# pdh930105/ARCQuant

Hardware: AMD Instinct MI355X
Metric: ARC-NVFP4 GEMM TFLOP/s (M=4096, N=KQ=4096, KE=64) (higher is better)
Workload: dtype f16

## Files before the change

### arcquant_amd/csrc/gemm_tile.hip

```cpp
#include <hip/hip_runtime.h>
#include <stdint.h>
#include <stdlib.h>

#include <type_traits>

#include "arcq_internal.hpp"
#include "gemm_common.hpp"
#include "gemm_tile_common.hpp"

namespace arcq {

#ifdef ARCQ_STREAM_STAMPS
static unsigned long long* g_tile_stamps = nullptr;
#ifndef ARCQ_TILE_REPACKED_UNIT
extern "C" void arcq_debug_set_tile_stamps(void* p) { g_tile_stamps = reinterpret_cast<unsigned long long*>(p); }
#endif
#define ARCQ_TILE_STAMP(k)                                                                                     \
  do {                                                                                                         \
    if (p.stamps && tid == 0) {                                                                                \
      unsigned long long t0_, t1_;                                                                             \
      asm volatile("s_memtime %0\n\ts_memrealtime %1\n\ts_waitcnt lgkmcnt(0)" : "=s"(t0_), "=s"(t1_)::"memory"); \
      p.stamps[(size_t)blockIdx.x * (2 * kTileStamps) + 2 * (k)] = t0_;                                        \
      p.stamps[(size_t)blockIdx.x * (2 * kTileStamps) + 2 * (k) + 1] = t1_;                                    \
    }                                                                                                          \
  } while (0)
#else
#define ARCQ_TILE_STAMP(k) do { } while (0)
#endif

#ifndef ARCQ_TILE_WIDE_STORES
#define ARCQ_TILE_WIDE_STORES 1
#endif

template <int BM, int BN, int WAVES_M, int WAVES_N, bool kMfma32, int kEpi, bool kStagger, bool kPipe, int kBLayout = kBRef>
__global__ __launch_bounds__(WAVES_M* WAVES_N * 64) void gemm_tile_kernel(TileParams p) {
  constexpr int kThreads = WAVES_M * WAVES_N * 64;
  constexpr int WM = BM / WAVES_M, WN = BN / WAVES_N;
  constexpr int kT = kMfma32 ? 32 : 16;
  constexpr int TM = WM / kT, TN = WN / kT;
  using acc_t = typename std::conditional<kMfma32, f32x16, f32x4>::type;
  constexpr int A_UNITS = (BM * 2 + kThreads - 1) / kThreads, B_UNITS = (BN * 2 + kThreads - 1) / kThreads;
  constexpr bool A_PARTIAL = (BM * 2) % kThreads != 0, B_PARTIAL = (BN * 2) % kThreads != 0;
  static_assert(!A_PARTIAL || A_UNITS == 1, "a partial A pass is a single pass");
  static_assert(!B_PARTIAL || B_UNITS == 1, "a partial B pass is a single pass");
  constexpr int A_TILE = BM * kRowBytes, B_TILE = BN * kRowBytes;

  extern __shared__ __attribute__((aligned(16))) unsigned char smem[];
  unsigned char* const lds_a0 = smem;
  unsigned char* const lds_b0 = smem + A_TILE;
  unsigned char* const lds_a1 = smem + A_TILE + B_TILE;
  unsigned char* const lds_b1 = smem + 2 * A_TILE + B_TILE;

  const int ntiles = p.tiles_m * p.tiles_n;
  int bid = blockIdx.x, split = 0;
  if (p.splits > 1) {
    split = bid / ntiles;
    bid -= split * ntiles;
  }
  {
    const int q8 = ntiles >> 3, r8 = ntiles & 7, x = bid & 7, j = bid >> 3;
    bid = (x < r8 ? x * (q8 + 1) : r8 * (q8 + 1) + (x - r8) * q8) + j;
  }
  constexpr int kGroupM = 8;
  const int per_group = kGroupM * p.tiles_n;
  const int grp = bid / per_group;
  const int first_m = grp * kGroupM;
  const int gsz = min(p.tiles_m - first_m, kGroupM);
  const int tm = first_m + (bid % per_group) % gsz;
  const int tn = (bid % per_group) / gsz;
  const int m0 = __builtin_amdgcn_readfirstlane(tm * BM), n0 = __builtin_amdgcn_readfirstlane(tn * BN);

  const int tid = threadIdx.x;
  const int lane = tid & 63, wave = tid >> 6;
  const int wr = wave / WAVES_N, wc = wave % WAVES_N;
  ARCQ_TILE_STAMP(0);
  const int half_k = p.K >> 1, atoms_k = p.K >> 6;
  const int a_begin = split * p.atoms_per_split, a_end = min(atoms_k, a_begin + p.atoms_per_split);

  const uint8_t* a_q[A_UNITS];
  const uint8_t* a_sf[A_UNITS];
  uint32_t a_live[A_UNITS];
  int a_slot[A_UNITS][4];
#pragma unroll
  for (int u = 0; u < A_UNITS; ++u) {
    const int unit = tid + u * kThreads, r = A_PARTIAL ? min(unit >> 1, BM - 1) : unit >> 1, h = unit & 1;
    const int row = m0 + r, rc = row < p.M ? row : p.M - 1;
    a_q[u] = p.A + (size_t)rc * half_k + h * 16;
    a_sf[u] = p.SFA + sf_atom_offset(rc, 0, atoms_k) + h * 2;
    a_live[u] = row < p.M ? 0xffffu : 0u;
#pragma unroll
    for (int j = 0; j < 4; ++j) a_slot[u][j] = kMfma32 ? lds_slot32(r, h * 4 + j) : lds_slot(r, h * 4 + j);
  }
  const uint8_t* b_q[B_UNITS];
  const uint8_t* b_sf[B_UNITS];
  uint32_t b_live[B_UNITS];
  int b_slot[B_UNITS][4];
#pragma unroll
  for (int u = 0; u < B_UNITS; ++u) {
    const int unit = tid + u * kThreads, r = B_PARTIAL ? min(unit >> 1, BN - 1) : unit >> 1, h = unit & 1;
    const int row = n0 + r, rc = row < p.N ? row : p.N - 1;
    if constexpr (kBLayout == kBRepacked) {
      const int tiles = ((p.K + 255) >> 8) * 2;
      b_q[u] = p.B + (size_t)(rc >> 4) * tiles * 1024 + h * 256 + (rc & 15) * 16;
      b_sf[u] = p.SFB + (size_t)(rc >> 4) * tiles * 128 + h * 64 + (rc & 15) * 4;
    } else {
      b_q[u] = p.B + (size_t)rc * half_k + h * 16;
      b_sf[u] = p.SFB + sf_atom_offset(rc, 0, atoms_k) + h * 2;
    }
    b_live[u] = row < p.N ? 0xffffu : 0u;
#pragma unroll
    for (int j = 0; j < 4; ++j) b_slot[u][j] = kMfma32 ? lds_slot32(r, h * 4 + j) : lds_slot(r, h * 4 + j);
  }
  const int fa_base = kMfma32 ? lds_slot32(wr * WM + (lane & 31), lane >> 5) : lds_slot(wr * WM + (lane & 15), lane >> 4);
  const int fb_base = kMfma32 ? lds_slot32(wc * WN + (lane & 31), lane >> 5) : lds_slot(wc * WN + (lane & 15), lane >> 4);
  acc_t acc[TM][TN];
#pragma unroll
  for (int i = 0; i < TM; ++i)
#pragma unroll
    for (int j = 0; j < TN; ++j)
#pragma unroll
      for (int r = 0; r < (kMfma32 ? 16 : 4); ++r) acc[i][j][r] = 0.f;

  Staged sa[A_UNITS], sb[B_UNITS];
  auto load_step = [&](int atom) {
#pragma unroll
    for (int u = 0; u < A_UNITS; ++u) sa[u] = stage_load(a_q[u], a_sf[u], atom);
#pragma unroll
    for (int u = 0; u < B_UNITS; ++u) sb[u] = kBLayout == kBRepacked ? stage_load_rw(b_q[u], b_sf[u], atom) : stage_load(b_q[u], b_sf[u], atom);
  };
  auto store_step = [&](unsigned char* la, unsigned char* lb) {
#pragma unroll
    for (int u = 0; u < A_UNITS; ++u)
      if (!A_PARTIAL || tid < BM * 2) stage_store(la, a_slot[u], sa[u], a_live[u]);
#pragma unroll
    for (int u = 0; u < B_UNITS; ++u)
      if (!B_PARTIAL || tid < BN * 2) stage_store(lb, b_slot[u], sb[u], b_live[u]);
  };
  auto mma_step = [&](const unsigned char* la, const unsigned char* lb) {
    if constexpr (kMfma32) {
#pragma unroll
      for (int ks = 0; ks < 4; ++ks) {
        Frag8 fa[TM], fb[TN];
#pragma unroll
        for (int i = 0; i < TM; ++i) fa[i].u = *reinterpret_cast<const uint4*>(la + (fa_base ^ (ks * 32)) + i * 32 * kRowBytes);
#pragma unroll
        for (int j = 0; j < TN; ++j) fb[j].u = *reinterpret_cast<const uint4*>(lb + (fb_base ^ (ks * 32)) + j * 32 * kRowBytes);
#pragma unroll
        for (int i = 0; i < TM; ++i)
#pragma unroll
          for (int j = 0; j < TN; ++j) acc[i][j] = __builtin_amdgcn_mfma_f32_32x32x16_f16(fb[j].v, fa[i].v, acc[i][j], 0, 0, 0);
      }
    } else {
#pragma unroll
      for (int ks = 0; ks < 2; ++ks) {
        Frag8 fa[TM], fb[TN];
#pragma unroll
        for (int i = 0; i < TM; ++i) fa[i].u = *reinterpret_cast<const uint4*>(la + (fa_base ^ (ks * 64)) + i * 16 * kRowBytes);
#pragma unroll
        for (int j = 0; j < TN; ++j) fb[j].u = *reinterpret_cast<const uint4*>(lb + (fb_base ^ (ks * 64)) + j * 16 * kRowBytes);
#pragma unroll
        for (int i = 0; i < TM; ++i)
#pragma unroll
          for (int j = 0; j < TN; ++j) acc[i][j] = __builtin_amdgcn_mfma_f32_16x16x32_f16(fb[j].v, fa[i].v, acc[i][j], 0, 0, 0);
      }
    }
  };
  const bool late = kStagger && wave >= 4;
  auto k_step = [&](int kt, unsigned char* ca, unsigned char* cb, unsigned char* na, unsigned char* nb) {
    Staged ta[A_UNITS], tb[B_UNITS];
#pragma unroll
    for (int u = 0; u < A_UNITS; ++u) ta[u] = sa[u];
#pragma unroll
    for (int u = 0; u < B_UNITS; ++u) tb[u] = sb[u];
    load_step(min(kt + 2 + (late ? 1 : 0), a_end - 1));
    __builtin_amdgcn_sched_barrier(0);
    mma_step(ca, cb);
    if (kStagger && late) __syncthreads();
    unsigned char* const wa = late ? ca : na;
    unsigned char* const wb = late ? cb : nb;
#pragma unroll
    for (int u = 0; u < A_UNITS; ++u)
      if (!A_PARTIAL || tid < BM * 2) stage_store(wa, a_slot[u], ta[u], a_live[u]);
#pragma unroll
    for (int u = 0; u < B_UNITS; ++u)
      if (!B_PARTIAL || tid < BN * 2) stage_store(wb, b_slot[u], tb[u], b_live[u]);
    if (!kStagger || !late) __syncthreads();
  };

  auto k_step_pipe = [&](int kt, unsigned char* ca, unsigned char* cb, unsigned char* na, unsigned char* nb) {
    static_assert(kMfma32 || TM % 2 == 0, "pairs of A fragments");
    Staged ta[A_UNITS], tb[B_UNITS];
#pragma unroll
    for (int u = 0; u < A_UNITS; ++u) ta[u] = sa[u];
#pragma unroll
    for (int u = 0; u < B_UNITS; ++u) tb[u] = sb[u];
    load_step(min(kt + 2, a_end - 1));
    __builtin_amdgcn_sched_barrier(0);
    constexpr int kPieces = (A_UNITS + B_UNITS) * 4, kBlocks = kMfma32 ? 4 : TM;
    auto pieces = [&](int blk) {
#pragma unroll
      for (int c = blk; c < kPieces; c += kBlocks) {
        const int u = c >> 2, j = c & 3;
        if (u < A_UNITS) {
#ifdef ARCQ_EXPERIMENT_A_RAW
          if (!A_PARTIAL || tid < BM * 2) stage_piece_raw(na, a_slot[u < A_UNITS ? u : 0][j], ta[u < A_UNITS ? u : 0], a_live[u < A_UNITS ? u : 0], j);
#else
          if (!A_PARTIAL || tid < BM * 2) stage_piece(na, a_slot[u < A_UNITS ? u : 0][j], ta[u < A_UNITS ? u : 0], a_live[u < A_UNITS ? u : 0], j);
#endif
        } else {
          const int v = u - A_UNITS < B_UNITS ? u - A_UNITS : 0;
#ifdef ARCQ_EXPERIMENT_B_RAW
          if (!B_PARTIAL || tid < BN * 2) stage_piece_raw(nb, b_slot[v][j], tb[v], b_live[v], j);
#else
          if (!B_PARTIAL || tid < BN * 2) stage_piece(nb, b_slot[v][j], tb[v], b_live[v], j);
#endif
        }
      }
    };
    if constexpr (kMfma32) {
      Frag8 f32a[2][TM], f32b[2][TN];
      auto rd_set = [&](int buf, int ks) {
#pragma unroll
        for (int i = 0; i < TM; ++i) f32a[buf][i].u = *reinterpret_cast<const uint4*>(ca + (fa_base ^ (ks * 32)) + i * 32 * kRowBytes);
#pragma unroll
        for (int j = 0; j < TN; ++j) f32b[buf][j].u = *reinterpret_cast<const uint4*>(cb + (fb_base ^ (ks * 32)) + j * 32 * kRowBytes);
      };
      rd_set(0, 0);
#pragma unroll
      for (int ks = 0; ks < 4; ++ks) {
        if (ks + 1 < 4) rd_set((ks + 1) & 1, ks + 1);
        __builtin_amdgcn_sched_barrier(0);
#pragma unroll
        for (int i = 0; i < TM; ++i)
#pragma unroll
          for (int j = 0; j < TN; ++j)
            if constexpr (kMfma32)
              acc[i][j] = __builtin_amdgcn_mfma_f32_32x32x16_f16(f32b[ks & 1][j].v, f32a[ks & 1][i].v, acc[i][j], 0, 0, 0);
        pieces(ks);
        __builtin_amdgcn_sched_barrier(0);
      }
      __syncthreads();
      return;
    }
    auto rd_a = [&](int ks, int i) { Frag8 f; f.u = *reinterpret_cast<const uint4*>(ca + (fa_base ^ (ks * 64)) + i * 16 * kRowBytes); return f; };
    auto rd_b = [&](int ks, int j) { Frag8 f; f.u = *reinterpret_cast<const uint4*>(cb + (fb_base ^ (ks * 64)) + j * 16 * kRowBytes); return f; };
    constexpr int kPairs = TM / 2, kSeq = 2 * kPairs, kAhead = 1;
    Frag8 fb[2][TN], fq[kSeq][2];
    auto rd_pair = [&](int q) {
      fq[q][0] = rd_a(q / kPairs, 2 * (q % kPairs));
      fq[q][1] = rd_a(q / kPairs, 2 * (q % kPairs) + 1);
    };
#pragma unroll
    for (int j = 0; j < TN; ++j) fb[0][j] = rd_b(0, j);
#pragma unroll
    for (int q = 0; q < kAhead; ++q) rd_pair(q);
#pragma unroll
    for (int q = 0; q < kSeq; ++q) {
      const int ks = q / kPairs, pr = q % kPairs;
      if (q + kAhead < kSeq) rd_pair(q + kAhead);
      if (ks == 0 && pr == kPairs - 1 - (kAhead - 1 < kPairs - 1 ? kAhead - 1 : kPairs - 1)) {
#pragma unroll
        for (int j = 0; j < TN; ++j) fb[1][j] = rd_b(1, j);
      }
      __builtin_amdgcn_sched_barrier(0);
#pragma unroll
      for (int ii = 0; ii < 2; ++ii)
#pragma unroll
        for (int j = 0; j < TN; ++j)
          if constexpr (!kMfma32)
            acc[2 * pr + ii][j] = __builtin_amdgcn_mfma_f32_16x16x32_f16(fb[ks][j].v, fq[q][ii].v, acc[2 * pr + ii][j], 0, 0, 0);
      pieces(q);
#pragma unroll
      for (int m8 = 0; m8 < (TM == 8 ? 2 * TN : 0); ++m8) {
        __builtin_amdgcn_sched_group_barrier(0x008, 1, 0);
        __builtin_amdgcn_sched_group_barrier(0x002, 2, 0);
      }
      __builtin_amdgcn_sched_barrier(0);
    }
    __syncthreads();
  };

  load_step(a_begin);
  Staged sa0[A_UNITS], sb0[B_UNITS];
#pragma unroll
  for (int u = 0; u < A_UNITS; ++u) sa0[u] = sa[u];
#pragma unroll
  for (int u = 0; u < B_UNITS; ++u) sb0[u] = sb[u];
  load_step(min(a_begin + 1, a_end - 1));
  __builtin_amdgcn_sched_barrier(0);
#pragma unroll
  for (int u = 0; u < A_UNITS; ++u)
    if (!A_PARTIAL || tid < BM * 2) stage_store(lds_a0, a_slot[u], sa0[u], a_live[u]);
#pragma unroll
  for (int u = 0; u < B_UNITS; ++u)
    if (!B_PARTIAL || tid < BN * 2) stage_store(lds_b0, b_slot[u], sb0[u], b_live[u]);
  if (kStagger && late) {
    store_step(lds_a1, lds_b1);
    load_step(min(a_begin + 2, a_end - 1));
  }
  __syncthreads();
  int kt = a_begin;
#ifndef ARCQ_EXPERIMENT_GENERAL_EPILOGUE
  float alpha_dev = 1.0f;
  if (p.alpha_dev) alpha_dev = *reinterpret_cast<const __attribute__((address_space(4))) float*>(reinterpret_cast<uintptr_t>(p.alpha_dev));
  asm volatile("" : "+s"(alpha_dev));
#endif
  if (WAVES_M * WAVES_N == 8 && wave >= 4) __builtin_amdgcn_s_setprio(1);
  ARCQ_TILE_STAMP(1);
  if constexpr (kPipe) {
    for (; kt + 1 < a_end; kt += 2) {
      k_step_pipe(kt, lds_a0, lds_b0, lds_a1, lds_b1);
      k_step_pipe(kt + 1, lds_a1, lds_b1, lds_a0, lds_b0);
    }
    if (kt < a_end) k_step_pipe(kt, lds_a0, lds_b0, lds_a1, lds_b1);
  } else {
    for (; kt + 1 < a_end; kt += 2) {
      k_step(kt, lds_a0, lds_b0, lds_a1, lds_b1);
      k_step(kt + 1, lds_a1, lds_b1, lds_a0, lds_b0);
    }
    if (kt < a_end) k_step(kt, lds_a0, lds_b0, lds_a1, lds_b1);
  }
  ARCQ_TILE_STAMP(2);

#ifdef ARCQ_EXPERIMENT_GENERAL_EPILOGUE
  const float alpha = p.alpha_host * (p.alpha_dev ? *p.alpha_dev : 1.0f);
#else
  const float alpha = p.alpha_host * alpha_dev;
#endif
  const bool vec_ok = (p.N & 3) == 0;
  uint32_t act_max = 0;
  [[maybe_unused]] auto interior_epilogue = [&](auto has_bias, auto has_res) __attribute__((always_inline)) {
    constexpr bool kBias = decltype(has_bias)::value, kRes = decltype(has_res)::value;
    constexpr bool kSilu = kEpi == kEpiSiluMul;
    constexpr uint32_t kElem = kSilu ? 1 : 2;
    unsigned char* const tile_d = reinterpret_cast<unsigned char*>(p.D) + ((size_t)m0 * p.N + n0) * kElem;
    const unsigned char* const tile_r = kRes ? reinterpret_cast<const unsigned char*>(p.residual) + ((size_t)m0 * p.N + n0) * 2 : nullptr;
    uint32_t t = tid;
    asm volatile("" : "+v"(t));
    const uint32_t lane_row = (t >> 6) / WAVES_N * WM + (t & 15), lane_col = (t >> 6) % WAVES_N * WN + 4 * ((t >> 4) & 3);
    uint32_t off = lane_row * (uint32_t)p.N + lane_col;
    const uint32_t row_step = 16u * (uint32_t)p.N;
    constexpr bool kWide = ARCQ_TILE_WIDE_STORES && !kSilu && TN % 2 == 0;
    typedef uint32_t u32x4_a8 __attribute__((ext_vector_type(4), aligned(8)));
    [[maybe_unused]] const uint32_t g4 = (t >> 4) & 3;
    [[maybe_unused]] uint32_t off_w = off - 4 * g4 + ((g4 & 1) ? 16 + 4 * (g4 - 1) : 4 * g4);
    [[maybe_unused]] uint2 held = make_uint2(0, 0);
    float bias_f[TN][4];
    if constexpr (kBias) {
#pragma unroll
      for (int j = 0; j < TN; ++j) {
        const uint2 b = *reinterpret_cast<const uint2*>(p.bias + n0 + lane_col + j * 16);
        bias_f[j][0] = bf16_bits_to_f32(b.x & 0xffffu); bias_f[j][1] = bf16_bits_to_f32(b.x >> 16);
        bias_f[j][2] = bf16_bits_to_f32(b.y & 0xffffu); bias_f[j][3] = bf16_bits_to_f32(b.y >> 16);
      }
    }
    uint2 res_cur[TN], res_nxt[TN];
    auto res_load = [&](uint32_t o, uint2 (&r)[TN]) {
#pragma unroll
      for (int j = 0; j < TN; ++j) r[j] = *reinterpret_cast<const uint2*>(tile_r + (size_t)o * 2 + j * 32);
    };
    if constexpr (kRes) res_load(off, res_cur);
#pragma unroll
    for (int i = 0; i < TM; ++i) {
      if constexpr (kRes) { if (i + 1 < TM) res_load(off + row_step, res_nxt); }
#pragma unroll
      for (int j = 0; j < TN; ++j) {
        float d[4] = {alpha * acc[i][j][0], alpha * acc[i][j][1], alpha * acc[i][j][2], alpha * acc[i][j][3]};
        if constexpr (kSilu) {
          if constexpr (kBias) {
#pragma unroll
            for (int r = 0; r < 4; r += 2) {
              round2_to_bf16(d[r], d[r + 1]);
              d[r] += bias_f[j][r];
              d[r + 1] += bias_f[j][r + 1];
            }
          }
          const uint32_t y01 = pack_bf16x2_hw(d[0], d[1]), y23 = pack_bf16x2_hw(d[2], d[3]);
          const uint32_t a0 = silu_mul_bf16(y01 & 0xffffu, y01 >> 16), a1 = silu_mul_bf16(y23 & 0xffffu, y23 >> 16);
          *reinterpret_cast<uint32_t*>(tile_d + (size_t)off + j * 16) = a0 | (a1 << 16);
          act_max = max(act_max, max(a0 & 0x7fffu, a1 & 0x7fffu));
        } else {
          if constexpr (kBias) {
#pragma unroll
            for (int r = 0; r < 4; r += 2) {
              round2_to_bf16(d[r], d[r + 1]);
              d[r] += bias_f[j][r];
              d[r + 1] += bias_f[j][r + 1];
            }
          }
          if constexpr (kRes) {
            const uint32_t rw[2] = {res_cur[j].x, res_cur[j].y};
#pragma unroll
            for (int r = 0; r < 4; r += 2) {
              round2_to_bf16(d[r], d[r + 1]);
              d[r] += bf16_bits_to_f32(rw[r >> 1] & 0xffffu);
              d[r + 1] += bf16_bits_to_f32(rw[r >> 1] >> 16);
            }
          }
          const uint2 pk = make_uint2(pack_bf16x2_hw(d[0], d[1]), pack_bf16x2_hw(d[2], d[3]));
          if constexpr (kWide) {
            if (j & 1) {
              const auto lo = __builtin_amdgcn_permlane16_swap(held.x, pk.x, false, false);
              const auto hi = __builtin_amdgcn_permlane16_swap(held.y, pk.y, false, false);
              const u32x4_a8 v = {lo[0], hi[0], lo[1], hi[1]};
              *reinterpret_cast<u32x4_a8*>(tile_d + (size_t)off_w * 2 + (j >> 1) * 64) = v;
            } else {
              held = pk;
            }
          } else {
            *reinterpret_cast<uint2*>(tile_d + (size_t)off * 2 + j * 32) = pk;
          }
        }
        if (i == 0 && j == 0) ARCQ_TILE_STAMP(3);
      }
      if constexpr (kRes) {
#pragma unroll
        for (int j = 0; j < TN; ++j) res_cur[j] = res_nxt[j];
      }
      off += row_step;
      off_w += row_step;
    }
  };
  auto store4 = [&](int m, int n, float d0, float d1, float d2, float d3, bool pre, uint2 bias2, uint2 res2) __attribute__((always_inline)) {
    if (m >= p.M || n >= p.N) return;
    const uint32_t bw[2] = {bias2.x, bias2.y}, rw[2] = {res2.x, res2.y};
    auto bias_at = [&](int r) { return bf16_bits_to_f32(pre ? (bw[r >> 1] >> (16 * (r & 1))) & 0xffffu : (uint32_t)p.bias[n + r]); };
    if (kEpi == kEpiSiluMul) {
      uint32_t y[4] = {f32_to_bf16_bits(alpha * d0), f32_to_bf16_bits(alpha * d1), f32_to_bf16_bits(alpha * d2), f32_to_bf16_bits(alpha * d3)};
      if (p.bias) {
#pragma unroll
        for (int e = 0; e < 4; ++e) y[e] = f32_to_bf16_bits(bf16_bits_to_f32(y[e]) + bias_at(e));
      }
      const uint32_t a0 = silu_mul_bf16(y[0], y[1]);
      const uint32_t a1 = silu_mul_bf16(y[2], y[3]);
      *reinterpret_cast<uint32_t*>(reinterpret_cast<uint16_t*>(p.D) + (size_t)m * (p.N >> 1) + (n >> 1)) = a0 | (a1 << 16);
      act_max = max(act_max, max(a0 & 0x7fffu, a1 & 0x7fffu));
      return;
    }
    if (p.splits > 1) {
      *reinterpret_cast<float4*>(p.partial + ((size_t)split * p.M + m) * p.N + n) = make_float4(d0, d1, d2, d3);
      return;
    }
    float d[4] = {alpha * d0, alpha * d1, alpha * d2, alpha * d3};
    if (p.bias) {
#pragma unroll
      for (int r = 0; r < 4; ++r)
        if (pre || n + r < p.N) d[r] = (p.out_dtype == ARCQ_OUT_F32 ? d[r] : bf16_bits_to_f32(f32_to_bf16_bits(d[r]))) + bias_at(r);
    }
    if (p.residual) {
#pragma unroll
      for (int r = 0; r < 4; ++r)
        if (pre || n + r < p.N) {
          const float res = bf16_bits_to_f32(pre ? (rw[r >> 1] >> (16 * (r & 1))) & 0xffffu : (uint32_t)p.residual[(size_t)m * p.N + n + r]);
          d[r] = (p.out_dtype == ARCQ_OUT_F32 ? d[r] : bf16_bits_to_f32(f32_to_bf16_bits(d[r]))) + res;
        }
    }
    if (p.out_dtype == ARCQ_OUT_F32) {
      float* o = reinterpret_cast<float*>(p.D) + (size_t)m * p.N + n;
      if (vec_ok) *reinterpret_cast<float4*>(o) = make_float4(d[0], d[1], d[2], d[3]);
      else for (int r = 0; r < 4; ++r) if (n + r < p.N) o[r] = d[r];
    } else {
      uint16_t* o = reinterpret_cast<uint16_t*>(p.D) + (size_t)m * p.N + n;
      if (vec_ok) *reinterpret_cast<uint2*>(o) = make_uint2(pack_bf16x2(d[0], d[1]), pack_bf16x2(d[2], d[3]));
      else for (int r = 0; r < 4; ++r) if (n + r < p.N) o[r] = (uint16_t)f32_to_bf16_bits(d[r]);
    }
  };
#ifdef ARCQ_EXPERIMENT_GENERAL_EPILOGUE
  constexpr bool kInteriorPath = false;
#else
  constexpr bool kInteriorPath = !kMfma32;
#endif
  bool interior = false;
  if constexpr (kInteriorPath)
    interior = m0 + BM <= p.M && n0 + BN <= p.N && vec_ok && p.splits <= 1 && p.out_dtype == ARCQ_OUT_BF16 && (int64_t)BM * p.N < (1ll << 31) &&
               ((reinterpret_cast<uintptr_t>(p.bias) | reinterpret_cast<uintptr_t>(p.residual)) & 7) == 0;
  if (interior) {
    if constexpr (kInteriorPath) {
      using T = std::true_type;
      using F = std::false_type;
      if constexpr (kEpi == kEpiSiluMul) {
        if (p.bias) interior_epilogue(T{}, F{});
        else interior_epilogue(F{}, F{});
      } else if (p.bias) {
        if (p.residual) interior_epilogue(T{}, T{});
        else interior_epilogue(T{}, F{});
      } else {
        if (p.residual) interior_epilogue(F{}, T{});
        else interior_epilogue(F{}, F{});
      }
    }
  } else if constexpr (kMfma32) {
#pragma unroll
    for (int i = 0; i < TM; ++i)
#pragma unroll
      for (int j = 0; j < TN; ++j) {
        const int m = m0 + wr * WM + i * 32 + (lane & 31);
#pragma unroll
        for (int g = 0; g < 4; ++g) {
          const int n = n0 + wc * WN + j * 32 + 8 * g + 4 * (lane >> 5);
          store4(m, n, acc[i][j][4 * g + 0], acc[i][j][4 * g + 1], acc[i][j][4 * g + 2], acc[i][j][4 * g + 3], false, make_uint2(0, 0), make_uint2(0, 0));
        }
      }
  } else {
    const bool pre = vec_ok && p.splits <= 1 && ((reinterpret_cast<uintptr_t>(p.bias) | reinterpret_cast<uintptr_t>(p.residual)) & 7) == 0;
    const int nb = n0 + wc * WN + 4 * (lane >> 4), mb = m0 + wr * WM + (lane & 15);
    if (pre) {
      uint2 bias_v[TN], res_cur[TN], res_nxt[TN];
#pragma unroll
      for (int j = 0; j < TN; ++j) {
        bias_v[j] = res_cur[j] = res_nxt[j] = make_uint2(0, 0);
        if (p.bias && nb + j * 16 < p.N) bias_v[j] = *reinterpret_cast<const uint2*>(p.bias + nb + j * 16);
      }
      auto res_load = [&](int i, uint2 (&r)[TN]) {
        if (!p.residual) return;
        const int m = mb + i * 16;
#pragma unroll
        for (int j = 0; j < TN; ++j)
          if (m < p.M && nb + j * 16 < p.N) r[j] = *reinterpret_cast<const uint2*>(p.residual + (size_t)m * p.N + nb + j * 16);
      };
      res_load(0, res_cur);
#pragma unroll
      for (int i = 0; i < TM; ++i) {
        if (i + 1 < TM) res_load(i + 1, res_nxt);
#pragma unroll
        for (int j = 0; j < TN; ++j) {
          store4(mb + i * 16, nb + j * 16, acc[i][j][0], acc[i][j][1], acc[i][j][2], acc[i][j][3], true, bias_v[j], res_cur[j]);
          if (i == 0 && j == 0) ARCQ_TILE_STAMP(3);
        }
#pragma unroll
        for (int j = 0; j < TN; ++j) res_cur[j] = res_nxt[j];
      }
    } else {
#pragma unroll
      for (int i = 0; i < TM; ++i)
#pragma unroll
        for (int j = 0; j < TN; ++j) {
          store4(mb + i * 16, nb + j * 16, acc[i][j][0], acc[i][j][1], acc[i][j][2], acc[i][j][3], false, make_uint2(0, 0), make_uint2(0, 0));
          if (i == 0 && j == 0) ARCQ_TILE_STAMP(3);
        }
    }
  }
  ARCQ_TILE_STAMP(4);
  if (kEpi == kEpiSiluMul) {
    __shared__ uint32_t wave_max[WAVES_M * WAVES_N];
#pragma unroll
    for (int sh = 32; sh > 0; sh >>= 1) act_max = max(act_max, (uint32_t)__shfl_down((int)act_max, sh, 64));
    if (lane == 0) wave_max[wave] = act_max;
    __syncthreads();
    if (tid == 0) {
      uint32_t m = 0;
#pragma unroll
      for (int w = 0; w < WAVES_M * WAVES_N; ++w) m = max(m, wave_max[w]);
      p.slots[blockIdx.x] = m;
    }
  }
}

struct TileCfg { int id, bm, bn, waves; };
static constexpr TileCfg kTileCfgs[] = {{1, 128, 128, 4}, {2, 256, 256, 4}, {3, 256, 256, 8}, {4, 128, 256, 4}, {5, 256, 256, 8}, {6, 128, 128, 4},
                                        {7, 64, 256, 4}, {8, 32, 256, 4}, {9, 128, 128, 4}, {10, 128, 256, 8}, {11, 256, 128, 8}, {12, 128, 128, 8},
                                        {13, 64, 256, 8}, {14, 64, 128, 8}, {15, 64, 64, 4}, {16, 64, 128, 4}, {17, 128, 64, 4}};
static const TileCfg& tile_cfg(int id) {
  for (const TileCfg& c : kTileCfgs)
    if (c.id == id) return c;
  return kTileCfgs[2];
}

static int env_int(const char* name, int dflt) {
  const char* e = getenv(name);
  return e ? atoi(e) : dflt;
}
static int tile_cfg_override() {
  static const int v = env_int("ARCQ_TILE_CFG", 0);
  return v;
}
static int tile_split_override() {
  static const int v = env_int("ARCQ_TILE_SPLIT", 0);
  return v;
}
static bool tile_stagger() {
  static const int v = env_int("ARCQ_TILE_STAGGER", 0);
  return v != 0;
}
static bool tile_pipe() {
  static const int v = env_int("ARCQ_TILE_PIPE", 1);
  return v != 0;
}

static void tile_split(int64_t M, int64_t N, int64_t K, int BM, int BN, int* splits, int* atoms_per_split) {
  const int64_t tiles = ((M + BM - 1) / BM) * ((N + BN - 1) / BN);
  const int atoms = (int)(K / 64);
  int s = 1;
  if ((N % 4) == 0) {
    if (tile_split_override() > 0) s = min(tile_split_override(), max(atoms / 2, 1));
    else
      while (tiles * s < 256 && atoms / (s * 2) >= 8 && s < 32) s *= 2;
  }
  const int per = (atoms + s - 1) / s;
  *splits = (atoms + per - 1) / per;
  *atoms_per_split = per;
}

template <int BM, int BN, int WAVES_M, int WAVES_N, bool kMfma32 = false, int kEpi = kEpiPlain, int kBLayout = kBRef>
static int launch_tile(const GemmArgs& a, hipStream_t stream, bool allow_split = false) {
  TileParams p;
  p.A = a.A; p.B = a.B; p.SFA = a.SFA; p.SFB = a.SFB; p.D = a.D;
  p.alpha_dev = a.alpha_dev; p.bias = a.bias; p.residual = a.residual;
  p.M = a.M; p.N = a.N; p.K = a.K; p.alpha_host = a.alpha_host; p.out_dtype = a.out_dtype;
  p.tiles_m = (a.M + BM - 1) / BM;
  p.tiles_n = (a.N + BN - 1) / BN;
  p.splits = 1; p.atoms_per_split = a.K / 64; p.partial = nullptr;
  p.epi = a.epilogue; p.slots = a.absmax_slots;
#ifdef ARCQ_STREAM_STAMPS
  p.stamps = g_tile_stamps;
#endif
  if (allow_split && a.epilogue == kEpiPlain) {
    tile_split(a.M, a.N, a.K, BM, BN, &p.splits, &p.atoms_per_split);
    if (p.splits > 1) {
      const int64_t need = (int64_t)p.splits * a.M * a.N * (int64_t)sizeof(float);
      if (!a.workspace || a.workspace_bytes < need)
        return fail(ARCQ_ERR_WORKSPACE, "arcq_gemm_nvfp4: split-K needs %lld B of workspace, got %lld", (long long)need,
                    (long long)a.workspace_bytes);
      p.partial = reinterpret_cast<float*>(a.workspace);
    }
  }
  const size_t lds = 2 * (size_t)(BM + BN) * kRowBytes;
  constexpr bool kCanStagger = WAVES_M * WAVES_N == 8 && BM == 256 && BN == 256, kCanPipe = true;
  auto kern = gemm_tile_kernel<BM, BN, WAVES_M, WAVES_N, kMfma32, kEpi, false, false, kBLayout>;
  if (kCanPipe && tile_pipe()) kern = gemm_tile_kernel<BM, BN, WAVES_M, WAVES_N, kMfma32, kEpi, false, kCanPipe, kBLayout>;
  else if (kCanStagger && tile_stagger()) kern = gemm_tile_kernel<BM, BN, WAVES_M, WAVES_N, kMfma32, kEpi, kCanStagger, false, kBLayout>;
  static LdsOptIn lds_opt[3];
  const int which = (kCanPipe && tile_pipe()) ? 1 : (kCanStagger && tile_stagger()) ? 2 : 0;
  if (int rc = ensure_dynamic_lds(reinterpret_cast<const void*>(kern), lds_opt[which], (int)lds, "arcq_gemm_nvfp4 (tile)")) return rc;
  hipLaunchKernelGGL(kern, dim3((unsigned)(p.tiles_m * p.tiles_n * p.splits)), dim3(WAVES_M * WAVES_N * 64), lds, stream, p);
  hipError_t e = hipGetLastError();
  if (e != hipSuccess) return fail(ARCQ_ERR_LAUNCH, "arcq_gemm_nvfp4 (tile): launch failed: %s", hipGetErrorString(e));
  if (p.splits > 1) return gemm_splitk_finish(a, p.splits, stream);
  return ARCQ_OK;
}

static int tile_choice(int64_t M, int64_t N, int64_t K) {
  const int64_t t256 = ((M + 255) / 256) * ((N + 255) / 256);
  if (t256 >= 192) return 3;
  if (M <= 32) return 8;
  if (M <= 64) return 7;
  const int64_t t10 = ((M + 127) / 128) * ((N + 255) / 256);
  if (t10 <= 64 || t10 == 128 || (t10 > 224 && t10 <= 256) || (K >= 8192 && t10 >= 96 && t10 <= 256)) return 10;
  return 1;
}

static int effective_cfg(int64_t M, int64_t N, int64_t K, bool* may_split) {
  int id = tile_cfg_override();
  if (id == 0) id = tile_choice(M, N, K);
  id = tile_cfg(id).id;
  *may_split = !(id >= 2 && id <= 6) && id != 9;
  return id;
}

#ifndef ARCQ_TILE_REPACKED_UNIT
int64_t gemm_tile_silu_slots(int64_t M, int64_t N, int64_t K) {
  bool sp;
  const TileCfg& c = tile_cfg(effective_cfg(M, N, K, &sp));
  return ((M + c.bm - 1) / c.bm) * ((N + c.bn - 1) / c.bn);
}

int64_t gemm_tile_workspace_bytes(int64_t M, int64_t N, int64_t K) {
  int s = 1, per = 0;
  bool sp;
  const TileCfg& c = tile_cfg(effective_cfg(M, N, K, &sp));
  if (sp) tile_split(M, N, K, c.bm, c.bn, &s, &per);
  return s > 1 ? (int64_t)s * M * N * (int64_t)sizeof(float) : 0;
}
#endif

template <int kEpi, int kBLayout>
static int gemm_tile_epi(const GemmArgs& a, hipStream_t stream) {
  bool sp;
  switch (effective_cfg(a.M, a.N, a.K, &sp)) {
    case 1: case 9: return launch_tile<128, 128, 2, 2, false, kEpi, kBLayout>(a, stream, sp);
    case 2: return launch_tile<256, 256, 2, 2, false, kEpi, kBLayout>(a, stream);
    case 4: return launch_tile<128, 256, 2, 2, false, kEpi, kBLayout>(a, stream);
    case 5: return launch_tile<256, 256, 2, 4, true, kEpi, kBLayout>(a, stream);
    case 6: return launch_tile<128, 128, 2, 2, true, kEpi, kBLayout>(a, stream);
    case 7: return launch_tile<64, 256, 1, 4, false, kEpi, kBLayout>(a, stream, sp);
    case 8: return launch_tile<32, 256, 1, 4, false, kEpi, kBLayout>(a, stream, sp);
    case 10: return launch_tile<128, 256, 2, 4, false, kEpi, kBLayout>(a, stream, sp);
    case 11: return launch_tile<256, 128, 4, 2, false, kEpi, kBLayout>(a, stream, sp);
    case 12: return launch_tile<128, 128, 2, 4, false, kEpi, kBLayout>(a, stream, sp);
    case 13: return launch_tile<64, 256, 1, 8, false, kEpi, kBLayout>(a, stream, sp);
    case 14: return launch_tile<64, 128, 2, 4, false, kEpi, kBLayout>(a, stream, sp);
    case 15: return launch_tile<64, 64, 2, 2, false, kEpi, kBLayout>(a, stream, sp);
    case 16: return launch_tile<64, 128, 2, 2, false, kEpi, kBLayout>(a, stream, sp);
    case 17: return launch_tile<128, 64, 2, 2, false, kEpi, kBLayout>(a, stream, sp);
    default: return launch_tile<256, 256, 2, 4, false, kEpi, kBLayout>(a, stream);
  }
}

#ifndef ARCQ_TILE_REPACKED_UNIT
int gemm_tile(const GemmArgs& a, hipStream_t stream) {
  if (a.b_layout == kBRepacked) return gemm_tile_repacked(a, stream);
  return a.epilogue == kEpiSiluMul ? gemm_tile_epi<kEpiSiluMul, kBRef>(a, stream) : gemm_tile_epi<kEpiPlain, kBRef>(a, stream);
}
#else
int gemm_tile_repacked(const GemmArgs& a, hipStream_t stream) {
  return a.epilogue == kEpiSiluMul ? gemm_tile_epi<kEpiSiluMul, kBRepacked>(a, stream) : gemm_tile_epi<kEpiPlain, kBRepacked>(a, stream);
}
#endif

}
```

### arcquant_amd/csrc/gemm_tile_common.hpp

```cpp
#pragma once
#include <hip/hip_runtime.h>
#include <stdint.h>

#include "arcq_internal.hpp"
#include "gemm_common.hpp"

namespace arcq {

struct TileParams {
  const uint8_t* A;
  const uint8_t* B;
  const uint8_t* SFA;
  const uint8_t* SFB;
  void* D;
  const float* alpha_dev;
  const uint16_t* bias;
  const uint16_t* residual;
  int M, N, K;
  float alpha_host;
  int out_dtype;
  int tiles_m, tiles_n;
  int splits, atoms_per_split;
  float* partial;
  int epi;
  unsigned int* slots;
#ifdef ARCQ_STREAM_STAMPS
  unsigned long long* stamps;
#endif
};
constexpr int kTileStamps = 5;

constexpr int kBK = 64;
constexpr int kRowBytes = kBK * 2;

__device__ __forceinline__ int lds_slot(int r, int ks) { return r * kRowBytes + ((ks ^ (r & 7)) << 4); }
__device__ __forceinline__ int lds_slot32(int r, int ks) { return r * kRowBytes + ((ks ^ ((r >> 1) & 7)) << 4); }

struct Staged {
  uint4 q;
  uint32_t sf;
};

__device__ __forceinline__ Staged stage_load(const uint8_t* __restrict__ qrow, const uint8_t* __restrict__ sfrow, int atom) {
  Staged s;
  s.q = *reinterpret_cast<const uint4*>(qrow + (size_t)atom * 32);
  s.sf = *reinterpret_cast<const uint16_t*>(sfrow + (size_t)atom * 512);
  return s;
}

__device__ __forceinline__ Staged stage_load_rw(const uint8_t* __restrict__ qrow, const uint8_t* __restrict__ sfrow, int atom) {
  Staged s;
  s.q = *reinterpret_cast<const uint4*>(qrow + (size_t)atom * 512);
  s.sf = *reinterpret_cast<const uint16_t*>(sfrow + (atom >> 2) * 256 + (atom & 1) * 128 + ((atom >> 1) & 1) * 2);
  return s;
}

__device__ __forceinline__ void stage_piece(unsigned char* tile, int slot, const Staged& s, uint32_t live_mask, int j) {
  const uint32_t w = j == 0 ? s.q.x : j == 1 ? s.q.y : j == 2 ? s.q.z : s.q.w;
  const Frag8 f = dequant8(w, sf_pair_at(s.sf & live_mask, j < 2 ? 0 : 8));
  *reinterpret_cast<uint4*>(tile + slot) = f.u;
}

#if defined(ARCQ_EXPERIMENT_A_RAW) || defined(ARCQ_EXPERIMENT_B_RAW)
__device__ __forceinline__ void stage_piece_raw(unsigned char* tile, int slot, const Staged& s, uint32_t live_mask, int j) {
  const uint32_t w = (j == 0 ? s.q.x : j == 1 ? s.q.y : j == 2 ? s.q.z : s.q.w) & (live_mask | (live_mask << 16)) & 0x3bff3bffu;
  *reinterpret_cast<uint4*>(tile + slot) = make_uint4(w, w, w, w);
}
#endif

__device__ __forceinline__ void stage_store(unsigned char* tile, const int (&slot)[4], const Staged& s, uint32_t live_mask) {
  const uint32_t sf = s.sf & live_mask;
  const f16x2 s0 = sf_pair_at(sf, 0), s1 = sf_pair_at(sf, 8);
  Frag8 f0 = dequant8(s.q.x, s0), f1 = dequant8(s.q.y, s0), f2 = dequant8(s.q.z, s1), f3 = dequant8(s.q.w, s1);
  *reinterpret_cast<uint4*>(tile + slot[0]) = f0.u;
  *reinterpret_cast<uint4*>(tile + slot[1]) = f1.u;
  *reinterpret_cast<uint4*>(tile + slot[2]) = f2.u;
  *reinterpret_cast<uint4*>(tile + slot[3]) = f3.u;
}


}
```

Measured before the change: 1404.

## Peel K-loop tail steps to drop redundant loads, stores and barriers

Restructures the main K loop for the non-stagger paths so the last two iterations are peeled into NoLoad and Last variants. The steady-state step no longer clamps the prefetch atom with min(), the NoLoad step skips global prefetch, and the Last step skips LDS staging and the trailing barrier. This removes wasted loads, dequant stores and a sync at the end of each tile. It also adds asm register pins so the scale-factor mask and fragment offsets are not rematerialized. The cost is more code, since several step variants are inlined, which may raise instruction-cache or register pressure.

```diff
diff --git a/arcquant_amd/csrc/gemm_tile.hip b/arcquant_amd/csrc/gemm_tile.hip
--- a/arcquant_amd/csrc/gemm_tile.hip
+++ b/arcquant_amd/csrc/gemm_tile.hip
@@ -136,15 +136,15 @@
     for (int u = 0; u < B_UNITS; ++u)
       if (!B_PARTIAL || tid < BN * 2) stage_store(lb, b_slot[u], sb[u], b_live[u]);
   };
-  auto mma_step = [&](const unsigned char* la, const unsigned char* lb) {
+  auto mma_step = [&](const unsigned char* la, const unsigned char* lb, int fa_off, int fb_off) {
     if constexpr (kMfma32) {
 #pragma unroll
       for (int ks = 0; ks < 4; ++ks) {
         Frag8 fa[TM], fb[TN];
 #pragma unroll
-        for (int i = 0; i < TM; ++i) fa[i].u = *reinterpret_cast<const uint4*>(la + (fa_base ^ (ks * 32)) + i * 32 * kRowBytes);
-#pragma unroll
-        for (int j = 0; j < TN; ++j) fb[j].u = *reinterpret_cast<const uint4*>(lb + (fb_base ^ (ks * 32)) + j * 32 * kRowBytes);
+        for (int i = 0; i < TM; ++i) fa[i].u = *reinterpret_cast<const uint4*>(la + (fa_off ^ (ks * 32)) + i * 32 * kRowBytes);
+#pragma unroll
+        for (int j = 0; j < TN; ++j) fb[j].u = *reinterpret_cast<const uint4*>(lb + (fb_off ^ (ks * 32)) + j * 32 * kRowBytes);
 #pragma unroll
         for (int i = 0; i < TM; ++i)
 #pragma unroll
@@ -155,9 +155,9 @@
       for (int ks = 0; ks < 2; ++ks) {
         Frag8 fa[TM], fb[TN];
 #pragma unroll
-        for (int i = 0; i < TM; ++i) fa[i].u = *reinterpret_cast<const uint4*>(la + (fa_base ^ (ks * 64)) + i * 16 * kRowBytes);
-#pragma unroll
-        for (int j = 0; j < TN; ++j) fb[j].u = *reinterpret_cast<const uint4*>(lb + (fb_base ^ (ks * 64)) + j * 16 * kRowBytes);
+        for (int i = 0; i < TM; ++i) fa[i].u = *reinterpret_cast<const uint4*>(la + (fa_off ^ (ks * 64)) + i * 16 * kRowBytes);
+#pragma unroll
+        for (int j = 0; j < TN; ++j) fb[j].u = *reinterpret_cast<const uint4*>(lb + (fb_off ^ (ks * 64)) + j * 16 * kRowBytes);
 #pragma unroll
         for (int i = 0; i < TM; ++i)
 #pragma unroll
@@ -165,16 +165,30 @@
       }
     }
   };
+  constexpr int kSteady = 0, kNoLoad = 1, kLast = 2;
+  using Steady = std::integral_constant<int, kSteady>;
+  using NoLoad = std::integral_constant<int, kNoLoad>;
+  using Last = std::integral_constant<int, kLast>;
+  auto next_atom = [](int kt) {
+    int atom = kt + 2;
+    asm volatile("" : "+s"(atom));
+    return atom;
+  };
   const bool late = kStagger && wave >= 4;
-  auto k_step = [&](int kt, unsigned char* ca, unsigned char* cb, unsigned char* na, unsigned char* nb) {
+  auto k_step = [&](auto tail, int kt, unsigned char* ca, unsigned char* cb, unsigned char* na, unsigned char* nb) __attribute__((always_inline)) {
+    constexpr int kTail = kStagger ? kSteady : decltype(tail)::value;
     Staged ta[A_UNITS], tb[B_UNITS];
 #pragma unroll
     for (int u = 0; u < A_UNITS; ++u) ta[u] = sa[u];
 #pragma unroll
     for (int u = 0; u < B_UNITS; ++u) tb[u] = sb[u];
-    load_step(min(kt + 2 + (late ? 1 : 0), a_end - 1));
+    if constexpr (kStagger) load_step(min(kt + 2 + (late ? 1 : 0), a_end - 1));
+    else if constexpr (kTail == kSteady) load_step(next_atom(kt));
     __builtin_amdgcn_sched_barrier(0);
-    mma_step(ca, cb);
+    int fa_off = fa_base, fb_off = fb_base;
+    if constexpr (kTail != kSteady) asm volatile("" : "+v"(fa_off), "+v"(fb_off));
+    mma_step(ca, cb, fa_off, fb_off);
+    if constexpr (kTail == kLast) return;
     if (kStagger && late) __syncthreads();
     unsigned char* const wa = late ? ca : na;
     unsigned char* const wb = late ? cb : nb;
@@ -187,16 +201,19 @@
     if (!kStagger || !late) __syncthreads();
   };
 
-  auto k_step_pipe = [&](int kt, unsigned char* ca, unsigned char* cb, unsigned char* na, unsigned char* nb) {
+  auto k_step_pipe = [&](auto tail, int kt, unsigned char* ca, unsigned char* cb, unsigned char* na, unsigned char* nb) __attribute__((always_inline)) {
     static_assert(kMfma32 || TM % 2 == 0, "pairs of A fragments");
+    constexpr int kTail = decltype(tail)::value;
     Staged ta[A_UNITS], tb[B_UNITS];
 #pragma unroll
     for (int u = 0; u < A_UNITS; ++u) ta[u] = sa[u];
 #pragma unroll
     for (int u = 0; u < B_UNITS; ++u) tb[u] = sb[u];
-    load_step(min(kt + 2, a_end - 1));
+    if constexpr (kTail == kSteady) load_step(next_atom(kt));
     __builtin_amdgcn_sched_barrier(0);
-    constexpr int kPieces = (A_UNITS + B_UNITS) * 4, kBlocks = kMfma32 ? 4 : TM;
+    int fa_off = fa_base, fb_off = fb_base;
+    if constexpr (kTail != kSteady) asm volatile("" : "+v"(fa_off), "+v"(fb_off));
+    constexpr int kPieces = kTail == kLast ? 0 : (A_UNITS + B_UNITS) * 4, kBlocks = kMfma32 ? 4 : TM;
     auto pieces = [&](int blk) {
 #pragma unroll
       for (int c = blk; c < kPieces; c += kBlocks) {
@@ -221,9 +238,9 @@
       Frag8 f32a[2][TM], f32b[2][TN];
       auto rd_set = [&](int buf, int ks) {
 #pragma unroll
-        for (int i = 0; i < TM; ++i) f32a[buf][i].u = *reinterpret_cast<const uint4*>(ca + (fa_base ^ (ks * 32)) + i * 32 * kRowBytes);
-#pragma unroll
-        for (int j = 0; j < TN; ++j) f32b[buf][j].u = *reinterpret_cast<const uint4*>(cb + (fb_base ^ (ks * 32)) + j * 32 * kRowBytes);
+        for (int i = 0; i < TM; ++i) f32a[buf][i].u = *reinterpret_cast<const uint4*>(ca + (fa_off ^ (ks * 32)) + i * 32 * kRowBytes);
+#pragma unroll
+        for (int j = 0; j < TN; ++j) f32b[buf][j].u = *reinterpret_cast<const uint4*>(cb + (fb_off ^ (ks * 32)) + j * 32 * kRowBytes);
       };
       rd_set(0, 0);
 #pragma unroll
@@ -239,11 +256,11 @@
         pieces(ks);
         __builtin_amdgcn_sched_barrier(0);
       }
-      __syncthreads();
+      if constexpr (kTail != kLast) __syncthreads();
       return;
     }
-    auto rd_a = [&](int ks, int i) { Frag8 f; f.u = *reinterpret_cast<const uint4*>(ca + (fa_base ^ (ks * 64)) + i * 16 * kRowBytes); return f; };
-    auto rd_b = [&](int ks, int j) { Frag8 f; f.u = *reinterpret_cast<const uint4*>(cb + (fb_base ^ (ks * 64)) + j * 16 * kRowBytes); return f; };
+    auto rd_a = [&](int ks, int i) { Frag8 f; f.u = *reinterpret_cast<const uint4*>(ca + (fa_off ^ (ks * 64)) + i * 16 * kRowBytes); return f; };
+    auto rd_b = [&](int ks, int j) { Frag8 f; f.u = *reinterpret_cast<const uint4*>(cb + (fb_off ^ (ks * 64)) + j * 16 * kRowBytes); return f; };
     constexpr int kPairs = TM / 2, kSeq = 2 * kPairs, kAhead = 1;
     Frag8 fb[2][TN], fq[kSeq][2];
     auto rd_pair = [&](int q) {
@@ -271,13 +288,13 @@
             acc[2 * pr + ii][j] = __builtin_amdgcn_mfma_f32_16x16x32_f16(fb[ks][j].v, fq[q][ii].v, acc[2 * pr + ii][j], 0, 0, 0);
       pieces(q);
 #pragma unroll
-      for (int m8 = 0; m8 < (TM == 8 ? 2 * TN : 0); ++m8) {
+      for (int m8 = 0; m8 < (TM == 8 && kTail != kLast ? 2 * TN : 0); ++m8) {
         __builtin_amdgcn_sched_group_barrier(0x008, 1, 0);
         __builtin_amdgcn_sched_group_barrier(0x002, 2, 0);
       }
       __builtin_amdgcn_sched_barrier(0);
     }
-    __syncthreads();
+    if constexpr (kTail != kLast) __syncthreads();
   };
 
   load_step(a_begin);
@@ -299,7 +316,6 @@
     load_step(min(a_begin + 2, a_end - 1));
   }
   __syncthreads();
-  int kt = a_begin;
 #ifndef ARCQ_EXPERIMENT_GENERAL_EPILOGUE
   float alpha_dev = 1.0f;
   if (p.alpha_dev) alpha_dev = *reinterpret_cast<const __attribute__((address_space(4))) float*>(reinterpret_cast<uintptr_t>(p.alpha_dev));
@@ -307,19 +323,37 @@
 #endif
   if (WAVES_M * WAVES_N == 8 && wave >= 4) __builtin_amdgcn_s_setprio(1);
   ARCQ_TILE_STAMP(1);
-  if constexpr (kPipe) {
-    for (; kt + 1 < a_end; kt += 2) {
-      k_step_pipe(kt, lds_a0, lds_b0, lds_a1, lds_b1);
-      k_step_pipe(kt + 1, lds_a1, lds_b1, lds_a0, lds_b0);
-    }
-    if (kt < a_end) k_step_pipe(kt, lds_a0, lds_b0, lds_a1, lds_b1);
-  } else {
-    for (; kt + 1 < a_end; kt += 2) {
-      k_step(kt, lds_a0, lds_b0, lds_a1, lds_b1);
-      k_step(kt + 1, lds_a1, lds_b1, lds_a0, lds_b0);
-    }
-    if (kt < a_end) k_step(kt, lds_a0, lds_b0, lds_a1, lds_b1);
-  }
+  auto k_loop = [&](auto& step) __attribute__((always_inline)) {
+    int kt = a_begin;
+    if constexpr (kStagger) {
+      for (; kt + 1 < a_end; kt += 2) {
+        step(Steady{}, kt, lds_a0, lds_b0, lds_a1, lds_b1);
+        step(Steady{}, kt + 1, lds_a1, lds_b1, lds_a0, lds_b0);
+      }
+      if (kt < a_end) step(Steady{}, kt, lds_a0, lds_b0, lds_a1, lds_b1);
+    } else {
+      for (; kt + 3 < a_end; kt += 2) {
+        step(Steady{}, kt, lds_a0, lds_b0, lds_a1, lds_b1);
+        step(Steady{}, kt + 1, lds_a1, lds_b1, lds_a0, lds_b0);
+      }
+      const int left = a_end - kt;
+      if (left == 3) {
+        step(Steady{}, kt, lds_a0, lds_b0, lds_a1, lds_b1);
+        ++kt;
+      }
+      unsigned char* ca = left == 3 ? lds_a1 : lds_a0;
+      unsigned char* na = left == 3 ? lds_a0 : lds_a1;
+      if (left >= 2) {
+        step(NoLoad{}, kt, ca, ca + A_TILE, na, na + A_TILE);
+        ca = na;
+      }
+      int once = 1;
+      asm volatile("" : "+s"(once));
+      for (int t = 0; t < once; ++t) step(Last{}, a_end - 1, ca, ca + A_TILE, na, na + A_TILE);
+    }
+  };
+  if constexpr (kPipe) k_loop(k_step_pipe);
+  else k_loop(k_step);
   ARCQ_TILE_STAMP(2);
 
 #ifdef ARCQ_EXPERIMENT_GENERAL_EPILOGUE
diff --git a/arcquant_amd/csrc/gemm_tile_common.hpp b/arcquant_amd/csrc/gemm_tile_common.hpp
--- a/arcquant_amd/csrc/gemm_tile_common.hpp
+++ b/arcquant_amd/csrc/gemm_tile_common.hpp
@@ -57,7 +57,9 @@
 
 __device__ __forceinline__ void stage_piece(unsigned char* tile, int slot, const Staged& s, uint32_t live_mask, int j) {
   const uint32_t w = j == 0 ? s.q.x : j == 1 ? s.q.y : j == 2 ? s.q.z : s.q.w;
-  const Frag8 f = dequant8(w, sf_pair_at(s.sf & live_mask, j < 2 ? 0 : 8));
+  uint32_t sf = s.sf & live_mask;
+  asm("" : "+v"(sf));
+  const Frag8 f = dequant8(w, sf_pair_at(sf, j < 2 ? 0 : 8));
   *reinterpret_cast<uint4*>(tile + slot) = f.u;
 }
 
```

New measurement: 1398. About the same (-0.4%).
